# DIAGNijmegen/prostateMR_3D-CAD-csPCa

Measured on AMD Instinct MI355X. Metric: train-step volumes/sec (whole job), M1 (20,160,160,3), higher is better.
Workload: dtype bf16; 1 GPU; C3 M1 full hierarchical-probabilistic dense_skip+deep_supervision latents (3,2,1,0) (20,160,160,3); batch_per_gpu=2, global_batch=2, params=67254246, parallelism=dp1, hip_graph=True

## Files before the change

prostatemr_3d-cad-cspca_amd/csrc/conv_halo.hip:

```cpp
#include "conv_mfma.h"
#include "reduce.h"
#include <stdlib.h>
#include <stdio.h>

#define HL_MAX_XIT 10
#define HL_MAX_CH 18

struct HaloP {
    MfmaP m;
    int TW, TH, tiles_w, tiles_h, ntiles, nsplit;
    int KDs, IHt, IWt;
    int dmin, hmin, wmin;
    int sde, she, swe, pde, phe, pwe;
    int PX, spr;
    int x_slots, x_bytes;
    int nchunks, nseg, kpad;
    int b_bytes, c_bytes, stages;
    int BNh;
    int nthr;
    int tiles_per_sample;
    int spr_sh, tw_sh;
    int ncls;
    int QH, QW;
};

__device__ __forceinline__ int x_swz(int row, int sl, int spr) {
    return spr == 8 ? (sl ^ (row & 7)) : (spr == 4 ? (sl ^ ((row >> 1) & 3)) : sl);
}

__device__ __forceinline__ unsigned long long gload8_untracked(const void* p) {
    unsigned long long v;
    asm volatile("global_load_dwordx2 %0, %1, off" : "=&v"(v) : "v"(p) : "memory");
    return v;
}

template <int TN, int NTHR, int NCH, int NXIT, int B1 = 0, int B2 = 0, int B3 = 0>
__global__ void __launch_bounds__(NTHR) conv_halo_kernel(HaloP p) {
    constexpr int TM = 2, BN = TN * 16, SEG = 8, NW = NTHR / 64;
    constexpr bool RT = NCH == 0;
    constexpr bool CLS = B1 > 0;
    constexpr int NC = CLS ? 4 : 1;
    static_assert(!CLS || (NCH > 0 && B1 < B2 && B2 < B3 && B3 < NCH), "class boundaries");
#define cls_of(ch) (CLS ? ((ch) >= B1) + ((ch) >= B2) + ((ch) >= B3) : 0)
#define cls_lo(c) ((c) == 0 ? 0 : ((c) == 1 ? B1 : ((c) == 2 ? B2 : B3)))
    constexpr int CH = RT ? HL_MAX_CH : NCH, XIT = RT ? HL_MAX_XIT : NXIT;
    extern __shared__ __attribute__((aligned(16))) unsigned char smem[];
    unsigned char* const Bs = smem;
    float* const red = reinterpret_cast<float*>(smem + p.b_bytes);
    unsigned char* const Xs0 = smem + p.b_bytes + p.c_bytes;
    const MfmaP& m = p.m;
    const int tid = threadIdx.x, lane = tid & 63, wave = __builtin_amdgcn_readfirstlane(tid >> 6);
    const int oc0 = blockIdx.x * BN;
    const unsigned char* zero_pg = reinterpret_cast<const unsigned char*>(m1_zero_page);
    const int fr = lane & 15, fs = lane >> 4;
    const int spt_sh = p.spr_sh;

    {
        const bf16_t* wp = (const bf16_t*)m.wp + m.cls_woff[0];
        const int nslot = p.nchunks * BN * 4;
        for (int q0 = 0; q0 < nslot; q0 += NTHR) {
            const int q = q0 + tid;
            const int ch = q / (BN * 4), r = (q / 4) % BN, s = m1_swz64(r, q & 3);
            const unsigned char* src;
            if constexpr (CLS) {
                const int c = cls_of(ch), lo = cls_lo(c), kp = m.cls_kpad[c];
                src = (q < nslot) ? reinterpret_cast<const unsigned char*>((const bf16_t*)m.wp + m.cls_woff[c] + (long long)(oc0 + r) * kp + ((ch - lo) * 4 + s) * SEG) : zero_pg;
            } else
            src = (q < nslot) ? reinterpret_cast<const unsigned char*>(wp + (long long)(oc0 + r) * p.kpad + (ch * 4 + s) * SEG)
                                                   : zero_pg;
            if (q0 + wave * 64 < nslot) m1_glds16(src, Bs + (q0 + wave * 64) * 16);
        }
    }

    const bf16_t* x_ptr[XIT]; int x_C[XIT], x_pk[XIT];
    const int nxit = RT ? p.x_slots / NTHR : NXIT;
    const int nchunks = RT ? p.nchunks : NCH;
    const int x_rows = p.KDs * p.IHt * p.IWt;
#pragma unroll
    for (int it = 0; it < XIT; ++it) {
        const int q = it * NTHR + tid;
        const int row = q >> spt_sh, slp = q & (p.spr - 1);
        const int sl = x_swz(row, slp, p.spr);
        const int dd = row / (p.IHt * p.IWt); const int r2 = row - dd * (p.IHt * p.IWt);
        const int hh = r2 / p.IWt, ww = r2 - hh * p.IWt;
        int c = sl * SEG, s = 0;
        while (s < m.nsrc - 1 && c >= m.srcC[s]) { c -= m.srcC[s]; ++s; }
        x_C[it] = m.srcC[s];
        x_ptr[it] = (const bf16_t*)m.src[s] + (long long)((dd * m.IH + hh) * m.IW + ww) * m.srcC[s] + c;
        x_pk[it] = row < x_rows ? (dd | (hh << 8) | (ww << 16)) : -1;
    }

    int q_kt = blockIdx.y, q_tw, q_th, q_od, q_n;
    { int r = q_kt; q_tw = r % p.tiles_w; r /= p.tiles_w; q_th = r % p.tiles_h; r /= p.tiles_h; q_od = r % m.OD; q_n = r / m.OD; }
    int s_tw, s_th, s_od, s_n;
    { int r = p.nsplit; s_tw = r % p.tiles_w; r /= p.tiles_w; s_th = r % p.tiles_h; r /= p.tiles_h; s_od = r % m.OD; s_n = r / m.OD; }
    auto advance = [&](int& kt, int& tw, int& th, int& od, int& n) {
        kt += p.nsplit;
        tw += s_tw; int c = tw >= p.tiles_w; tw -= c ? p.tiles_w : 0;
        th += s_th + c; c = th >= p.tiles_h; th -= c ? p.tiles_h : 0;
        od += s_od + c; c = od >= m.OD; od -= c ? m.OD : 0;
        n += s_n + c;
    };
    auto issue = [&](int st) {
        const int live = q_kt < p.ntiles;
        const int id0 = q_od * p.sde - p.pde + p.dmin, ih0 = q_th * p.TH * p.she - p.phe + p.hmin, iw0 = q_tw * p.TW * p.swe - p.pwe + p.wmin;
        const int lin0 = ((q_n * m.ID + id0) * m.IH + ih0) * m.IW + iw0;
        unsigned char* Xs = Xs0 + st * p.x_bytes;
        const long long zp = (long long)zero_pg;
        const bool inside = live && id0 >= 0 && id0 + p.KDs <= m.ID && ih0 >= 0 && ih0 + p.IHt <= m.IH && iw0 >= 0 && iw0 + p.IWt <= m.IW;
        if (inside) {
#pragma unroll
            for (int it = 0; it < XIT; ++it) {
                if (!RT || it < nxit) {
                    const long long real = (long long)(x_ptr[it] + (long long)lin0 * x_C[it]);
                    const int ok = x_pk[it] >= 0;
                    const unsigned char* src = reinterpret_cast<const unsigned char*>(zp + ((real - zp) & -(long long)ok));
                    m1_glds16(src, Xs + (it * NTHR + wave * 64) * 16);
                }
            }
        } else {
#pragma unroll
            for (int it = 0; it < XIT; ++it) {
                if (!RT || it < nxit) {
                    const int pk = x_pk[it];
                    const int dd = pk & 0xff, hh = (pk >> 8) & 0xff, ww = (pk >> 16) & 0xff;
                    const int ok = live & (int)(pk >= 0) & (int)((unsigned)(id0 + dd) < (unsigned)m.ID) & (int)((unsigned)(ih0 + hh) < (unsigned)m.IH) &
                                   (int)((unsigned)(iw0 + ww) < (unsigned)m.IW);
                    const long long real = (long long)(x_ptr[it] + (long long)lin0 * x_C[it]);
                    const unsigned char* src = reinterpret_cast<const unsigned char*>(zp + ((real - zp) & -(long long)ok));
                    m1_glds16(src, Xs + (it * NTHR + wave * 64) * 16);
                }
            }
        }
        advance(q_kt, q_tw, q_th, q_od, q_n);
    };

    const unsigned lds0 = (unsigned)(unsigned long long)(lptr_t)smem;
    const int tw_sh = p.tw_sh;
    unsigned a_off[CH][TM];
#pragma unroll
    for (int q = 0; q < CH; ++q) {
        int kseg = q * 4 + fs, t0 = 0;
        if constexpr (CLS) {
            const int c = cls_of(q);
            kseg = (q - cls_lo(c)) * 4 + fs; t0 = m.cls_first[c];
            if (kseg >= m.cls_ntaps[c] * p.spr) kseg = 0;
        } else if (kseg >= p.nseg) kseg = 0;
        const int t = t0 + (kseg >> spt_sh), sl = kseg & (p.spr - 1);
        const int ddr = m.tdd[t] - p.dmin, dhr = m.tdh[t] - p.hmin, dwr = m.tdw[t] - p.wmin;
#pragma unroll
        for (int i = 0; i < TM; ++i) {
            const int mv = wave * 32 + i * 16 + fr;
            const int th = mv >> tw_sh, tw = mv & (p.TW - 1);
            const int row = (ddr * p.IHt + th * p.she + dhr) * p.IWt + tw * p.swe + dwr;
            a_off[q][i] = lds0 + p.b_bytes + p.c_bytes + row * p.PX + x_swz(row, sl, p.spr) * 16;
        }
    }
    unsigned b_off[TN];
#pragma unroll
    for (int j = 0; j < TN; ++j) b_off[j] = lds0 + (j * 16 + fr) * 64 + m1_swz64(fr, fs) * 16;

    int e_th[TM], e_row[TM];
#pragma unroll
    for (int i = 0; i < TM; ++i) {
        const int mv = wave * 32 + i * 16 + fr;
        e_th[i] = mv >> tw_sh; e_row[i] = CLS ? 2 * (e_th[i] * m.OW + (mv & (p.TW - 1))) : e_th[i] * m.OW + (mv & (p.TW - 1));
    }
    bf16_t* o_base[TN]; int o_C[TN], o_nv[TN], o_acc[TN], o_fast[TN]; float bias_r[TN][4];
#pragma unroll
    for (int j = 0; j < TN; ++j) {
        const int oc = oc0 + j * 16 + fs * 4;
        int nv = m.OCn - oc; nv = nv > 4 ? 4 : (nv < 0 ? 0 : nv);
        o_base[j] = nullptr; o_C[j] = 0; o_acc[j] = 0; o_fast[j] = 0;
        if (nv > 0) {
            const OutRef o = m1_out_ref(m, oc);
            if (o.base) { o_base[j] = (bf16_t*)o.base + o.col; o_C[j] = o.C; o_acc[j] = o.acc; o_fast[j] = nv == 4 && (o.C & 3) == 0 && (o.col & 3) == 0; }
            else nv = 0;
        }
        o_nv[j] = nv;
#pragma unroll
        for (int r = 0; r < 4; ++r) bias_r[j][r] = (oc + r < m.OCn) ? m1_bias_at(m, oc + r) : 0.f;
    }
#pragma unroll
    for (int j = 0; j < TN; ++j)
#pragma unroll
        for (int r = 0; r < 4; ++r) asm volatile("" : "+v"(bias_r[j][r]));
    const bool ib = !CLS && m.ib_x != nullptr;
    float* const ib_ms = red + NW * BN * 2;
    float ib_g[TN][4], ib_b[TN][4];
#pragma unroll
    for (int j = 0; j < TN; ++j)
#pragma unroll
        for (int r = 0; r < 4; ++r) {
            const int oc = oc0 + j * 16 + fs * 4 + r;
            ib_g[j][r] = (ib && oc < m.OCn) ? m.ib_gamma[oc] : 0.f; ib_b[j][r] = (ib && oc < m.OCn) ? m.ib_beta[oc] : 0.f;
        }
    if (ib) {
        for (int e = tid; e < m.N * BN; e += NTHR) {
            const int n = e / BN, c = e - n * BN, oc = oc0 + c < m.OCn ? oc0 + c : 0;
            ib_ms[e * 2] = m.ib_stats[((long long)n * m.OC + oc) * 2]; ib_ms[e * 2 + 1] = m.ib_stats[((long long)n * m.OC + oc) * 2 + 1];
        }
    }
#pragma unroll
    for (int j = 0; j < TN; ++j)
#pragma unroll
        for (int r = 0; r < 4; ++r) asm volatile("" : "+v"(ib_g[j][r]), "+v"(ib_b[j][r]));
    if (ib) { asm volatile("s_waitcnt vmcnt(0)" ::: "memory"); __syncthreads(); }
    float ssum[TN][4], ssq[TN][4];
#pragma unroll
    for (int j = 0; j < TN; ++j)
#pragma unroll
        for (int r = 0; r < 4; ++r) { ssum[j][r] = 0.f; ssq[j][r] = 0.f; }
    int cur_n = 0;
    bool any_acc = false;
#pragma unroll
    for (int j = 0; j < TN; ++j) any_acc |= o_acc[j] != 0;
    any_acc = __builtin_amdgcn_readfirstlane(__any(any_acc)) != 0;
    const bool want_stats = !CLS && m.stat_partial != nullptr;
    auto flush = [&](int n) {
#pragma unroll
        for (int j = 0; j < TN; ++j)
#pragma unroll
            for (int r = 0; r < 4; ++r) {
                float s = ssum[j][r], q = ssq[j][r];
#pragma unroll
                for (int o = 1; o < 16; o <<= 1) { s += __shfl_xor(s, o); q += __shfl_xor(q, o); }
                if (fr == 0) { red[(wave * BN + j * 16 + fs * 4 + r) * 2] = s; red[(wave * BN + j * 16 + fs * 4 + r) * 2 + 1] = q; }
                ssum[j][r] = 0.f; ssq[j][r] = 0.f;
            }
        __syncthreads();
        if (tid < BN && oc0 + tid < m.OCn) {
            float s = 0.f, q = 0.f;
            for (int w = 0; w < NW; ++w) { s += red[(w * BN + tid) * 2]; q += red[(w * BN + tid) * 2 + 1]; }
            float* dst = m.stat_partial + (((long long)n * p.nsplit + blockIdx.y) * m.OC + oc0 + tid) * 2;
            dst[0] = s; dst[1] = q;
        }
        __syncthreads();
    };

    const int S = p.stages, npiece = nxit;
    int c_kt = blockIdx.y, c_tw = q_tw, c_th = q_th, c_od = q_od, c_n = q_n;
    for (int s = 0; s < S - 1; ++s) issue(s);
    int st = 0;
    for (; c_kt < p.ntiles; advance(c_kt, c_tw, c_th, c_od, c_n)) {
        if (want_stats) { for (; cur_n < c_n; ++cur_n) flush(cur_n); }
        if constexpr (RT) m1_wait_vm<40>(npiece * (S - 2));
        else { if (S == 2) m1_wait_vm_imm<0>(); else if (S == 3) m1_wait_vm_imm<NXIT>(); else m1_wait_vm_imm<2 * NXIT>(); }
        __builtin_amdgcn_s_barrier();
        const int oh0 = c_th * p.TH;
        const int row0 = CLS ? ((c_n * m.OD + c_od) * m.OH + 2 * oh0) * m.OW + 2 * c_tw * p.TW
                             : ((c_n * m.OD + c_od) * m.OH + oh0) * m.OW + c_tw * p.TW;
        unsigned long long oldv[NC][TM][TN], xv[TM][TN];
        if (ib) {
#pragma unroll
            for (int i = 0; i < TM; ++i)
#pragma unroll
                for (int j = 0; j < TN; ++j) {
                    xv[i][j] = 0ull;
                    if (o_fast[j] && oh0 + e_th[i] < p.QH)
                        xv[i][j] = gload8_untracked((const bf16_t*)m.ib_x + (long long)(row0 + e_row[i]) * m.OC + oc0 + j * 16 + fs * 4);
                }
        }
        if (any_acc) {
#pragma unroll
            for (int c = 0; c < NC; ++c)
#pragma unroll
            for (int i = 0; i < TM; ++i)
#pragma unroll
                for (int j = 0; j < TN; ++j) {
                    oldv[c][i][j] = 0ull;
                    if (o_acc[j] && o_fast[j] && oh0 + e_th[i] < p.QH)
                        oldv[c][i][j] = gload8_untracked(o_base[j] + (long long)(row0 + e_row[i] + (c >> 1) * m.OW + (c & 1)) * o_C[j]);
                }
        }
        int stn = st + S - 1; if (stn >= S) stn -= S;
        issue(stn);
        const unsigned sb = (unsigned)(st * p.x_bytes);

        f32x4_t acc[NC][TM][TN];
#pragma unroll
        for (int c = 0; c < NC; ++c)
#pragma unroll
        for (int i = 0; i < TM; ++i)
#pragma unroll
            for (int j = 0; j < TN; ++j) acc[c][i][j] = (f32x4_t){0.f, 0.f, 0.f, 0.f};
        u32x4_t af[2][TM], bf[2][TN];
#pragma unroll
        for (int i = 0; i < TM; ++i) af[0][i] = m1_lds_read128(a_off[0][i] + sb);
#pragma unroll
        for (int j = 0; j < TN; ++j) bf[0][j] = m1_lds_read128(b_off[j]);
#pragma unroll
        for (int q = 0; q < CH; ++q) {
            if (!RT || q < nchunks) {
                const int cur = q & 1;
                m1_lds_wait(af[cur][0]);
#pragma unroll
                for (int i = 1; i < TM; ++i) m1_lds_tie(af[cur][i]);
#pragma unroll
                for (int j = 0; j < TN; ++j) m1_lds_tie(bf[cur][j]);
                if (q + 1 < CH && (!RT || q + 1 < nchunks)) {
#pragma unroll
                    for (int i = 0; i < TM; ++i) af[cur ^ 1][i] = m1_lds_read128(a_off[q + 1 < CH ? q + 1 : q][i] + sb);
#pragma unroll
                    for (int j = 0; j < TN; ++j) bf[cur ^ 1][j] = m1_lds_read128(b_off[j] + (q + 1) * BN * 64);
                }
                __builtin_amdgcn_sched_barrier(0);
#pragma unroll
                for (int i = 0; i < TM; ++i)
#pragma unroll
                    for (int j = 0; j < TN; ++j)
                        acc[cls_of(q)][i][j] = __builtin_amdgcn_mfma_f32_16x16x32_bf16(__builtin_bit_cast(bf16x8_t, bf[cur][j]),
                                                                            __builtin_bit_cast(bf16x8_t, af[cur][i]), acc[cls_of(q)][i][j], 0, 0, 0);
                __builtin_amdgcn_sched_barrier(0);
            }
        }

        if (any_acc || ib) {
            if constexpr (RT) m1_wait_vm_imm<0>(); else m1_wait_vm_imm<NXIT>();
#pragma unroll
            for (int i = 0; i < TM; ++i)
#pragma unroll
                for (int j = 0; j < TN; ++j) {
                    if (any_acc) {
#pragma unroll
                        for (int c = 0; c < NC; ++c) asm volatile("" : "+v"(oldv[c][i][j]));
// ... 62 lines not shown
    asm volatile("s_waitcnt vmcnt(0)" ::: "memory");
}
#undef cls_of
#undef cls_lo

typedef void (*halo_kern_t)(HaloP);
static halo_kern_t halo_cls_kernel(const MfmaP& mp, const HaloP& p) {
    const int nxit = p.x_slots / p.nthr;
    const int b1 = mp.cls_kpad[0] / 32, b2 = b1 + mp.cls_kpad[1] / 32, b3 = b2 + mp.cls_kpad[2] / 32;
    halo_kern_t kern = nullptr;
#define HC(NCH_, NXIT_, B1_, B2_, B3_) if (!kern && p.nchunks == NCH_ && nxit == NXIT_ && b1 == B1_ && b2 == B2_ && b3 == B3_) \
        kern = p.BNh == 32 ? conv_halo_kernel<2, 512, NCH_, NXIT_, B1_, B2_, B3_> : conv_halo_kernel<1, 512, NCH_, NXIT_, B1_, B2_, B3_>;
    HC(18, 5, 8, 12, 16) HC(18, 5, 2, 6, 10)
    HC(5, 2, 2, 3, 4) HC(5, 2, 1, 2, 3)
    HC(9, 3, 4, 6, 8) HC(9, 3, 1, 3, 5)
#undef HC
    return kern;
}
static bool halo_plan_nthr(const MfmaP& m, int OCpad, HaloP& p, int force_nthr);
static bool halo_plan(const MfmaP& m, int OCpad, HaloP& p) {
    if (halo_plan_nthr(m, OCpad, p, 0)) return true;
    return halo_plan_nthr(m, OCpad, p, 256);
}
static bool halo_plan_nthr(const MfmaP& m, int OCpad, HaloP& p, int force_nthr) {
    if (m.ksplit != 1) return false;
    const bool cls4 = m.mode == 1 && m.nclasses == 4 && m.sd == 1 && m.sh == 2 && m.sw == 2 && m.OH % 2 == 0 && m.OW % 2 == 0 &&
                      m.IH == m.OH / 2 && m.IW == m.OW / 2 && m.ID == m.OD && !m.stat_partial && !m.ib_x;
    { int hc = M1_CFG("M1_HALO_CLASSES", 1); if (cls4 && !hc) return false; }
    if (m.nclasses != 1 && !cls4) return false;
    if (!(m.mode == 0 || (m.mode == 1 && m.sd == 1 && m.sh == 1 && m.sw == 1) || cls4)) return false;
    { int hs = M1_CFG("M1_HALO_STRIDED", 1);
      if (!hs && m.mode == 0 && (m.sd > 1 || m.sh > 1 || m.sw > 1)) return false; }
    int CC = 0;
    for (int i = 0; i < m.nsrc; ++i) { if (m.srcC[i] % 8) return false; CC += m.srcC[i]; }
    if (!(CC == 8 || CC == 16 || CC == 32 || CC == 64)) return false;
    const int QH = cls4 ? m.OH / 2 : m.OH, QW = cls4 ? m.OW / 2 : m.OW;
    if (QW % 8) return false;
    if ((long long)m.N * m.ID * m.IH * m.IW >= (1ll << 31) - (1 << 20) || (long long)m.N * m.OD * m.OH * m.OW >= (1ll << 31) - (1 << 20)) return false;
    int nt = m.cls_ntaps[0];
    if (cls4) { nt = 0; for (int c = 0; c < 4; ++c) { if (m.cls_first[c] != nt) return false; nt += m.cls_ntaps[c]; } }
    if (nt < 2 || m.cls_first[0] != 0) return false;
    p = HaloP{}; p.m = m; p.ncls = cls4 ? 4 : 1; p.QH = QH; p.QW = QW;
    int dmin = 127, dmax = -127, hmin = 127, hmax = -127, wmin = 127, wmax = -127;
    for (int t = 0; t < nt; ++t) {
        dmin = m.tdd[t] < dmin ? m.tdd[t] : dmin; dmax = m.tdd[t] > dmax ? m.tdd[t] : dmax;
        hmin = m.tdh[t] < hmin ? m.tdh[t] : hmin; hmax = m.tdh[t] > hmax ? m.tdh[t] : hmax;
        wmin = m.tdw[t] < wmin ? m.tdw[t] : wmin; wmax = m.tdw[t] > wmax ? m.tdw[t] : wmax;
    }
    p.dmin = dmin; p.hmin = hmin; p.wmin = wmin;
    if (m.mode == 0) { p.sde = m.sd; p.she = m.sh; p.swe = m.sw; p.pde = m.pd; p.phe = m.ph; p.pwe = m.pw; }
    else { p.sde = p.she = p.swe = 1; p.pde = p.phe = p.pwe = 0; }
    { int nt_ = M1_CFG("M1_HALO_THREADS", 512); p.nthr = nt_ == 512 ? 512 : 256; }
    if (force_nthr) p.nthr = force_nthr;
    p.TW = QW % 32 == 0 ? 32 : (QW % 16 == 0 ? 16 : 8);
    if (p.nthr == 512) {
        const int th5 = 256 / p.TW, th2 = 128 / p.TW;
        const double e5 = (double)QH / ((QH + th5 - 1) / th5 * th5), e2 = (double)QH / ((QH + th2 - 1) / th2 * th2);
        if (e5 < 0.9 * e2) p.nthr = 256;
    }
    if (cls4 && p.nthr != 512) return false;
    const int BMh = p.nthr / 2;
    p.TH = BMh / p.TW;
    p.tiles_w = QW / p.TW; p.tiles_h = (QH + p.TH - 1) / p.TH;
    p.tiles_per_sample = m.OD * p.tiles_h * p.tiles_w;
    const long long nt_all = (long long)m.N * p.tiles_per_sample;
    if (nt_all >= (1ll << 30)) return false;
    p.ntiles = (int)nt_all;
    p.KDs = dmax - dmin + 1; p.IHt = (p.TH - 1) * p.she + (hmax - hmin + 1); p.IWt = (p.TW - 1) * p.swe + (wmax - wmin + 1);
    if (p.KDs > 255 || p.IHt > 255 || p.IWt > 255) return false;
    p.PX = CC * 2; p.spr = CC / 8;
    p.spr_sh = p.spr == 8 ? 3 : (p.spr == 4 ? 2 : (p.spr == 2 ? 1 : 0)); p.tw_sh = p.TW == 32 ? 5 : (p.TW == 16 ? 4 : 3);
    const int x_rows = p.KDs * p.IHt * p.IWt;
    p.x_slots = (x_rows * p.spr + p.nthr - 1) / p.nthr * p.nthr;
    if (p.x_slots > HL_MAX_XIT * p.nthr) return false;
    p.x_bytes = p.x_slots * 16 + 256;
    p.kpad = m.cls_kpad[0]; p.nchunks = p.kpad / 32; p.nseg = nt * p.spr;
    if (cls4) { p.kpad = 0; for (int c = 0; c < 4; ++c) p.kpad += m.cls_kpad[c]; p.nchunks = p.kpad / 32; }
    if (p.nchunks > HL_MAX_CH) return false;
    p.BNh = (m.OCn > 16 && OCpad >= 32) ? 32 : 16;
    if (OCpad % p.BNh) return false;
    p.b_bytes = p.nchunks * p.BNh * 64;
    p.c_bytes = (p.nthr / 64) * p.BNh * 2 * 4;
    if (m.ib_x) p.c_bytes += m.N * p.BNh * 2 * 4;
    const int fixed = p.b_bytes + p.c_bytes;
    int kb = M1_CFG("M1_HALO_LDS_KB", 160);
    int S = (kb * 1024 - fixed) / p.x_bytes;
    if (S > 4) S = 4;
    { int fs = M1_CFG("M1_HALO_STAGES", 0); if (fs >= 2 && fs < S) S = fs; }
    while (S > 2 && (p.x_slots / p.nthr) * (S - 2) > 40) --S;
    if (S < 2) return false;
    p.stages = S;
    if (cls4 && !halo_cls_kernel(m, p)) return false;
    return true;
}

static int halo_nsplit(const HaloP& p, int OCpad) {
    const int slices = OCpad / p.BNh;
    int nsplit = 256 / slices; if (nsplit < 1) nsplit = 1;
    { int tg = M1_CFG("M1_HALO_BLOCKS", 0); if (tg > 0) nsplit = tg / slices > 0 ? tg / slices : 1; }
    if (nsplit > p.ntiles) nsplit = p.ntiles;
    return nsplit;
}

bool m1_halo_conv_supported(const MfmaP& mp, int OCpad) { HaloP p; return halo_plan(mp, OCpad, p); }
int m1_halo_conv_stat_parts(const MfmaP& mp, int OCpad) { HaloP p; return halo_plan(mp, OCpad, p) ? halo_nsplit(p, OCpad) : 0; }

int m1_halo_conv(const MfmaP& mp, int OCpad, hipStream_t st) {
    HaloP p;
    if (!halo_plan(mp, OCpad, p)) return M1_ERR_UNSUPPORTED;
    const int slices = OCpad / p.BNh;
    const int nsplit = halo_nsplit(p, OCpad);
    p.nsplit = nsplit;
    if (mp.stat_partial && mp.stat_tiles != nsplit) return M1_ERR_BAD_ARG;
    const size_t smem = (size_t)p.b_bytes + p.c_bytes + (size_t)p.stages * p.x_bytes;
    const int nxit = p.x_slots / p.nthr;
    void (*kern)(HaloP) = nullptr;
    if (p.ncls == 4) {
        kern = halo_cls_kernel(mp, p);
        if (!kern) return M1_ERR_UNSUPPORTED;
    } else
    if (p.nthr == 512) {
#define HK(NCH_, NXIT_) if (!kern && p.nchunks == NCH_ && nxit == NXIT_) kern = p.BNh == 32 ? conv_halo_kernel<2, 512, NCH_, NXIT_> : conv_halo_kernel<1, 512, NCH_, NXIT_>;
        HK(18, 6) HK(9, 3) HK(5, 2) HK(3, 1) HK(14, 4) HK(7, 2)
#undef HK
    } else {
#define HK(NCH_, NXIT_) if (!kern && p.nchunks == NCH_ && nxit == NXIT_) kern = p.BNh == 32 ? conv_halo_kernel<2, 256, NCH_, NXIT_> : conv_halo_kernel<1, 256, NCH_, NXIT_>;
        HK(9, 9)
#undef HK
    }
    { int lg = M1_CFG("M1_HALO_LOG", 0);
      if (lg) fprintf(stderr, "halo: nthr %d BN %d nchunks %d nxit %d stages %d TW %d TH %d %s\n", p.nthr, p.BNh, p.nchunks, nxit, p.stages, p.TW, p.TH, kern ? "static" : "runtime"); }
    if (!kern) kern = p.nthr == 512 ? (p.BNh == 32 ? conv_halo_kernel<2, 512, 0, 0> : conv_halo_kernel<1, 512, 0, 0>)
                                    : (p.BNh == 32 ? conv_halo_kernel<2, 256, 0, 0> : conv_halo_kernel<1, 256, 0, 0>);
    if (m1_allow_dynamic_lds((const void*)kern, 160 * 1024) != M1_OK) return M1_ERR_LAUNCH;
    m1_note_kernel(p.ncls == 4 ? "conv_halo_cls:bn%d" : "conv_halo:bn%d", p.BNh);
    hipLaunchKernelGGL(kern, dim3(slices, nsplit), dim3(p.nthr), smem, st, p);
    return m1_check_launch();
}
```

prostatemr_3d-cad-cspca_amd/csrc/conv_mfma.h:

```cpp
#pragma once
#include "common.h"
#include "gather.h"
#include "cdna4.h"

#define MF_MAX_TAPS 27
#define MF_MAX_CLASSES 8

struct MfmaP {
    const void* src[M1_MAX_SRC];
    int srcC[M1_MAX_SRC];
    int srcSeg[M1_MAX_SRC];
    int nsrc, CC, spt;
    int ID, IH, IW;
    void* out;
    int OC, OCn;
    int nout;
    void* outs[M1_MAX_SRC]; int outC[M1_MAX_SRC]; int outOff[M1_MAX_SRC + 1]; int outAcc[M1_MAX_SRC];
    int OD, OH, OW, N;
    const void* wp;
    const float* bias;
    const float* bias2; int bias_split;
    int mode, sd, sh, sw, pd, ph, pw;
    int nclasses;
    int cls_ntaps[MF_MAX_CLASSES], cls_first[MF_MAX_CLASSES], cls_kpad[MF_MAX_CLASSES];
    long long cls_woff[MF_MAX_CLASSES];
    signed char tdd[MF_MAX_TAPS], tdh[MF_MAX_TAPS], tdw[MF_MAX_TAPS];
    int tap_pk[MF_MAX_TAPS];
    int accumulate;
    int ksplit;
    float* acc32;
    long long slab_elems;
    int aligned;
    int korder;
    const void* ib_x;
    const float* ib_stats; const float* ib_gamma; const float* ib_beta; float ib_slope;
    int tps;
    float* stat_partial;
    int stat_tiles;
};

struct OutRef { void* base; int C, col, acc; };
__device__ __forceinline__ OutRef m1_out_ref(const MfmaP& p, int oc) {
    if (p.nout == 0) return OutRef{p.out, p.OC, oc, p.accumulate};
    int m = 0;
    while (m + 1 < p.nout && oc >= p.outOff[m + 1]) ++m;
    return OutRef{p.outs[m], p.outC[m], oc - p.outOff[m], p.outAcc[m]};
}

__device__ __forceinline__ float m1_bias_at(const MfmaP& p, int oc) {
    if (p.bias_split > 0 && oc >= p.bias_split) return p.bias2 ? p.bias2[oc - p.bias_split] : 0.f;
    return p.bias ? p.bias[oc] : 0.f;
}

template <typename T> struct MT;
template <> struct MT<bf16_t> { static constexpr int SEG = 8; };
template <> struct MT<float> { static constexpr int SEG = 4; };


bool m1_halo_conv_supported(const MfmaP& mp, int OCpad);
int m1_halo_conv_stat_parts(const MfmaP& mp, int OCpad);
int m1_halo_conv(const MfmaP& mp, int OCpad, hipStream_t st);

bool m1_pw_conv_supported(const MfmaP& mp, int OCpad, int BN);
int m1_pw_conv_stat_parts(const MfmaP& mp, int OCpad, int BN);
int m1_pw_conv(const MfmaP& mp, int OCpad, int BN, hipStream_t st);
```

prostatemr_3d-cad-cspca_amd/csrc/conv_pw.hip:

```cpp
#include "conv_mfma.h"
#include "reduce.h"
#include <stdlib.h>


struct PwP {
    MfmaP m;
    int kpad, nseg;
    int nwaves;
    int V;
    long long Mtot;
};

template <int TN, int NCH>
__global__ void __launch_bounds__(256) conv_pw_kernel(PwP p) {
    constexpr int BN = TN * 16, NW = 4;
    extern __shared__ __attribute__((aligned(16))) unsigned char smem[];
    const MfmaP& m = p.m;
    const int tid = threadIdx.x, lane = tid & 63, wave = tid >> 6;
    const int fr = lane & 15, fs = lane >> 4;
    const int oc0 = blockIdx.x * BN;

    {
        const bf16_t* wp = (const bf16_t*)m.wp + m.cls_woff[0];
        for (int q = tid; q < NCH * BN * 4; q += 256) {
            const int ch = q / (BN * 4), r = (q / 4) % BN, s = q & 3;
            const uint4 v = *reinterpret_cast<const uint4*>(wp + (long long)(oc0 + r) * p.kpad + (ch * 4 + s) * 8);
            *reinterpret_cast<uint4*>(smem + ((ch * BN + r) * 4 + m1_swz64(r, s)) * 16) = v;
        }
    }
    __syncthreads();

    const bf16_t* xp[NCH]; int xC[NCH];
#pragma unroll
    for (int q = 0; q < NCH; ++q) {
        const int kseg = q * 4 + fs;
        int c = kseg * 8, s = 0;
        while (s < m.nsrc - 1 && c >= m.srcC[s]) { c -= m.srcC[s]; ++s; }
        const bool ok = kseg < p.nseg;
        xp[q] = ok ? (const bf16_t*)m.src[s] + c : nullptr; xC[q] = ok ? m.srcC[s] : 0;
    }
    bf16_t* o_base[TN]; int o_C[TN], o_nv[TN], o_acc[TN], o_fast[TN]; float bias_r[TN][4];
#pragma unroll
    for (int j = 0; j < TN; ++j) {
        const int oc = oc0 + j * 16 + fs * 4;
        int nv = m.OCn - oc; nv = nv > 4 ? 4 : (nv < 0 ? 0 : nv);
        o_base[j] = nullptr; o_C[j] = 0; o_acc[j] = 0; o_fast[j] = 0;
        if (nv > 0) {
            const OutRef o = m1_out_ref(m, oc);
            if (o.base) { o_base[j] = (bf16_t*)o.base + o.col; o_C[j] = o.C; o_acc[j] = o.acc; o_fast[j] = nv == 4 && (o.C & 3) == 0 && (o.col & 3) == 0; }
            else nv = 0;
        }
        o_nv[j] = nv;
#pragma unroll
        for (int r = 0; r < 4; ++r) bias_r[j][r] = (oc + r < m.OCn) ? m1_bias_at(m, oc + r) : 0.f;
    }
    const unsigned char* const w_rd = smem + fr * 64 + m1_swz64(fr, fs) * 16;

    const bool want_stats = m.stat_partial != nullptr;
    const bool ib = m.ib_x != nullptr;
    float ib_g[TN][4], ib_b[TN][4];
#pragma unroll
    for (int j = 0; j < TN; ++j)
#pragma unroll
        for (int r = 0; r < 4; ++r) {
            const int oc = oc0 + j * 16 + fs * 4 + r;
            ib_g[j][r] = (ib && oc < m.OCn) ? m.ib_gamma[oc] : 0.f; ib_b[j][r] = (ib && oc < m.OCn) ? m.ib_beta[oc] : 0.f;
        }
    float ssum[TN][4], ssq[TN][4];
#pragma unroll
    for (int j = 0; j < TN; ++j)
#pragma unroll
        for (int r = 0; r < 4; ++r) { ssum[j][r] = 0.f; ssq[j][r] = 0.f; }
    const int part = blockIdx.y * NW + wave;
    int cur_n = 0;
    auto flush = [&](int n) {
#pragma unroll
        for (int j = 0; j < TN; ++j)
#pragma unroll
            for (int r = 0; r < 4; ++r) {
                float s = ssum[j][r], q = ssq[j][r];
#pragma unroll
                for (int o = 1; o < 16; o <<= 1) { s += __shfl_xor(s, o); q += __shfl_xor(q, o); }
                const int oc = oc0 + j * 16 + fs * 4 + r;
                if (fr == 0 && oc < m.OCn) {
                    float* dst = m.stat_partial + (((long long)n * p.nwaves + part) * m.OC + oc) * 2;
                    dst[0] = s; dst[1] = q;
                }
                ssum[j][r] = 0.f; ssq[j][r] = 0.f;
            }
    };

    const long long step = (long long)p.nwaves * 32;
    u32x4_t xf[2][NCH], xn[2][NCH];
    auto fetch = [&](long long v0, u32x4_t (&x)[2][NCH]) {
#pragma unroll
        for (int i = 0; i < 2; ++i) {
            const long long v = v0 + i * 16 + fr;
#pragma unroll
            for (int q = 0; q < NCH; ++q) {
                x[i][q] = (u32x4_t){0u, 0u, 0u, 0u};
                if (v < p.Mtot && xp[q]) x[i][q] = *reinterpret_cast<const u32x4_t*>(xp[q] + v * xC[q]);
            }
        }
    };
    fetch((long long)part * 32, xf);
    for (long long v0 = (long long)part * 32; v0 < p.Mtot; v0 += step) {
        if (want_stats) { const int n = (int)(v0 / p.V); for (; cur_n < n; ++cur_n) flush(cur_n); }
        fetch(v0 + step, xn);
        bool vok[2];
#pragma unroll
        for (int i = 0; i < 2; ++i) vok[i] = v0 + i * 16 + fr < p.Mtot;
        f32x4_t acc[2][TN];
#pragma unroll
        for (int i = 0; i < 2; ++i)
#pragma unroll
            for (int j = 0; j < TN; ++j) acc[i][j] = (f32x4_t){0.f, 0.f, 0.f, 0.f};
#pragma unroll
        for (int q = 0; q < NCH; ++q)
#pragma unroll
            for (int j = 0; j < TN; ++j) {
                const u32x4_t wf = *reinterpret_cast<const u32x4_t*>(w_rd + (q * BN + j * 16) * 64);
#pragma unroll
                for (int i = 0; i < 2; ++i)
                    acc[i][j] = __builtin_amdgcn_mfma_f32_16x16x32_bf16(__builtin_bit_cast(bf16x8_t, wf), __builtin_bit_cast(bf16x8_t, xf[i][q]), acc[i][j], 0, 0, 0);
            }
#pragma unroll
        for (int i = 0; i < 2; ++i) {
            if (!vok[i]) continue;
            const long long orow = v0 + i * 16 + fr;
#pragma unroll
            for (int j = 0; j < TN; ++j) {
                if (o_nv[j] == 0) continue;
                bf16_t* dst = o_base[j] + orow * o_C[j];
                float v[4];
#pragma unroll
                for (int r = 0; r < 4; ++r) v[r] = acc[i][j][r] + bias_r[j][r];
                if (o_fast[j]) {
                    if (o_acc[j]) {
                        const uint2 ov = *reinterpret_cast<const uint2*>(dst);
                        const unsigned r01 = m1_cvt_pk_bf16(v[0], v[1]), r23 = m1_cvt_pk_bf16(v[2], v[3]);
                        v[0] = __uint_as_float(r01 << 16) + __uint_as_float(ov.x << 16); v[1] = __uint_as_float(r01 & 0xffff0000u) + __uint_as_float(ov.x & 0xffff0000u);
                        v[2] = __uint_as_float(r23 << 16) + __uint_as_float(ov.y << 16); v[3] = __uint_as_float(r23 & 0xffff0000u) + __uint_as_float(ov.y & 0xffff0000u);
                    }
                    uint2 o;
                    o.x = m1_cvt_pk_bf16(v[0], v[1]); o.y = m1_cvt_pk_bf16(v[2], v[3]);
                    *reinterpret_cast<uint2*>(dst) = o;
                    if (want_stats) {
                        const float r0 = __uint_as_float(o.x << 16), r1 = __uint_as_float(o.x & 0xffff0000u);
                        const float r2 = __uint_as_float(o.y << 16), r3 = __uint_as_float(o.y & 0xffff0000u);
                        if (ib) {
                            const int oc = oc0 + j * 16 + fs * 4, n = (int)(orow / p.V);
                            const float* msp = m.ib_stats + ((long long)n * m.OC + oc) * 2;
                            const float4 ms0 = *reinterpret_cast<const float4*>(msp), ms1 = *reinterpret_cast<const float4*>(msp + 4);
                            const uint2 xw = *reinterpret_cast<const uint2*>((const bf16_t*)m.ib_x + orow * m.OC + oc);
                            const float x0 = (__uint_as_float(xw.x << 16) - ms0.x) * ms0.y, x1 = (__uint_as_float(xw.x & 0xffff0000u) - ms0.z) * ms0.w;
                            const float x2 = (__uint_as_float(xw.y << 16) - ms1.x) * ms1.y, x3 = (__uint_as_float(xw.y & 0xffff0000u) - ms1.z) * ms1.w;
                            const float d0 = r0 * lrelu_g(ib_g[j][0] * x0 + ib_b[j][0], m.ib_slope), d1 = r1 * lrelu_g(ib_g[j][1] * x1 + ib_b[j][1], m.ib_slope);
                            const float d2 = r2 * lrelu_g(ib_g[j][2] * x2 + ib_b[j][2], m.ib_slope), d3 = r3 * lrelu_g(ib_g[j][3] * x3 + ib_b[j][3], m.ib_slope);
                            ssum[j][0] += d0; ssq[j][0] += d0 * x0; ssum[j][1] += d1; ssq[j][1] += d1 * x1;
                            ssum[j][2] += d2; ssq[j][2] += d2 * x2; ssum[j][3] += d3; ssq[j][3] += d3 * x3;
                        } else {
                        ssum[j][0] += r0; ssq[j][0] += r0 * r0; ssum[j][1] += r1; ssq[j][1] += r1 * r1;
                        ssum[j][2] += r2; ssq[j][2] += r2 * r2; ssum[j][3] += r3; ssq[j][3] += r3 * r3;
                        }
                    }
                } else {
#pragma unroll
                    for (int r = 0; r < 4; ++r)
                        if (r < o_nv[j]) {
                            float a = v[r];
                            if (o_acc[j]) a = bf2f(f2bf(a)) + bf2f(dst[r]);
                            const bf16_t e = f2bf(a); dst[r] = e;
                            const float vr = bf2f(e); ssum[j][r] += vr; ssq[j][r] += vr * vr;
                        }
                }
            }
        }
    #pragma unroll
        for (int i = 0; i < 2; ++i)
#pragma unroll
            for (int q = 0; q < NCH; ++q) xf[i][q] = xn[i][q];
    }
    if (want_stats) { for (; cur_n < m.N; ++cur_n) flush(cur_n); }
}

static bool pw_plan(const MfmaP& m, int OCpad, int BN, PwP& p) {
    int en = M1_CFG("M1_PW", 1);
    if (!en) return false;
    if (m.nclasses != 1 || m.ksplit != 1 || m.cls_ntaps[0] != 1) return false;
    if (m.tdd[0] != 0 || m.tdh[0] != 0 || m.tdw[0] != 0) return false;
    if (m.sd != 1 || m.sh != 1 || m.sw != 1) return false;
    if (m.ID != m.OD || m.IH != m.OH || m.IW != m.OW) return false;
    int CC = 0;
    for (int i = 0; i < m.nsrc; ++i) { if (m.srcC[i] % 8) return false; CC += m.srcC[i]; }
    const int kpad = m.cls_kpad[0];
    if (kpad % 32 || kpad / 32 > 2 || CC > kpad) return false;
    if (!(BN == 16 || BN == 32) || OCpad % BN) return false;
    p = PwP{}; p.m = m; p.kpad = kpad; p.nseg = CC / 8;
    p.V = m.OD * m.OH * m.OW; p.Mtot = (long long)m.N * p.V;
    if (p.V % 32) return false;
    return true;
}
static int pw_nwaves(const PwP& p, int OCpad, int BN) {
    const int slices = OCpad / BN;
    int tg = M1_CFG("M1_PW_BLOCKS", 2048);
    long long blocks = tg / slices; if (blocks < 1) blocks = 1;
    const long long need = (p.Mtot + 127) / 128;
    if (blocks > need) blocks = need;
    return (int)blocks * 4;
}
bool m1_pw_conv_supported(const MfmaP& mp, int OCpad, int BN) { PwP p; return pw_plan(mp, OCpad, BN, p); }
int m1_pw_conv_stat_parts(const MfmaP& mp, int OCpad, int BN) { PwP p; return pw_plan(mp, OCpad, BN, p) ? pw_nwaves(p, OCpad, BN) : 0; }

int m1_pw_conv(const MfmaP& mp, int OCpad, int BN, hipStream_t st) {
    PwP p;
    if (!pw_plan(mp, OCpad, BN, p)) return M1_ERR_UNSUPPORTED;
    p.nwaves = mp.stat_partial ? mp.stat_tiles : pw_nwaves(p, OCpad, BN);
    if (p.nwaves < 4 || p.nwaves % 4) return M1_ERR_BAD_ARG;
    const int nch = p.kpad / 32;
    const int NCH = nch <= 1 ? 1 : 2;
    if (NCH * 32 != p.kpad) {
        return M1_ERR_UNSUPPORTED;
    }
    void (*kern)(PwP) = nullptr;
#define PK(TN_, NCH_) if (BN == TN_ * 16 && NCH == NCH_) kern = conv_pw_kernel<TN_, NCH_>;
    PK(1, 1) PK(1, 2) PK(2, 1) PK(2, 2)
#undef PK
    if (!kern) return M1_ERR_UNSUPPORTED;
    const size_t smem = (size_t)NCH * BN * 64;
    if (smem > 48 * 1024 && m1_allow_dynamic_lds((const void*)kern, 64 * 1024) != M1_OK) return M1_ERR_LAUNCH;
    m1_note_kernel("conv_pw:bn%d", BN);
    hipLaunchKernelGGL(kern, dim3(OCpad / BN, p.nwaves / 4), dim3(256), smem, st, p);
    return m1_check_launch();
}
```

Baseline: 88.92 volumes/s.

## Stage kernel argument tables in LDS and issue prologue loads earlier

```diff
diff --git a/prostatemr_3d-cad-cspca_amd/csrc/conv_halo.hip b/prostatemr_3d-cad-cspca_amd/csrc/conv_halo.hip
--- a/prostatemr_3d-cad-cspca_amd/csrc/conv_halo.hip
+++ b/prostatemr_3d-cad-cspca_amd/csrc/conv_halo.hip
@@ -54,8 +54,23 @@
     const unsigned char* zero_pg = reinterpret_cast<const unsigned char*>(m1_zero_page);
     const int fr = lane & 15, fs = lane >> 4;
     const int spt_sh = p.spr_sh;
-
+    const bool ib = !CLS && m.ib_x != nullptr;
+
+    const MfmaTab* const tab = reinterpret_cast<const MfmaTab*>(smem + p.b_bytes + p.c_bytes - MF_TAB_BYTES);
+    float* const ib_ms = red + NW * BN * 2;
     {
+        const MfmaTabRow trow = m1_tab_load(m, tid, oc0, BN, ib);
+        if (ib) {
+            for (int e = tid; e < m.N * BN; e += NTHR) {
+                const int n = e / BN, c = e - n * BN, oc = oc0 + c < m.OCn ? oc0 + c : 0;
+                ib_ms[e * 2] = m.ib_stats[((long long)n * m.OC + oc) * 2]; ib_ms[e * 2 + 1] = m.ib_stats[((long long)n * m.OC + oc) * 2 + 1];
+            }
+        }
+        m1_tab_store(reinterpret_cast<MfmaTab*>(smem + p.b_bytes + p.c_bytes - MF_TAB_BYTES), trow, tid);
+    }
+    __syncthreads();
+
+    auto issue_weights = [&]() {
         const bf16_t* wp = (const bf16_t*)m.wp + m.cls_woff[0];
         const int nslot = p.nchunks * BN * 4;
         for (int q0 = 0; q0 < nslot; q0 += NTHR) {
@@ -63,14 +78,15 @@
             const int ch = q / (BN * 4), r = (q / 4) % BN, s = m1_swz64(r, q & 3);
             const unsigned char* src;
             if constexpr (CLS) {
-                const int c = cls_of(ch), lo = cls_lo(c), kp = m.cls_kpad[c];
-                src = (q < nslot) ? reinterpret_cast<const unsigned char*>((const bf16_t*)m.wp + m.cls_woff[c] + (long long)(oc0 + r) * kp + ((ch - lo) * 4 + s) * SEG) : zero_pg;
+                const int c = cls_of(ch), lo = cls_lo(c), kp = c == 0 ? m.cls_kpad[0] : (c == 1 ? m.cls_kpad[1] : (c == 2 ? m.cls_kpad[2] : m.cls_kpad[3]));
+                const long long wo = c == 0 ? m.cls_woff[0] : (c == 1 ? m.cls_woff[1] : (c == 2 ? m.cls_woff[2] : m.cls_woff[3]));
+                src = (q < nslot) ? reinterpret_cast<const unsigned char*>((const bf16_t*)m.wp + wo + (long long)(oc0 + r) * kp + ((ch - lo) * 4 + s) * SEG) : zero_pg;
             } else
             src = (q < nslot) ? reinterpret_cast<const unsigned char*>(wp + (long long)(oc0 + r) * p.kpad + (ch * 4 + s) * SEG)
                                                    : zero_pg;
             if (q0 + wave * 64 < nslot) m1_glds16(src, Bs + (q0 + wave * 64) * 16);
         }
-    }
+    };
 
     const bf16_t* x_ptr[XIT]; int x_C[XIT], x_pk[XIT];
     const int nxit = RT ? p.x_slots / NTHR : NXIT;
@@ -83,10 +99,9 @@
         const int sl = x_swz(row, slp, p.spr);
         const int dd = row / (p.IHt * p.IWt); const int r2 = row - dd * (p.IHt * p.IWt);
         const int hh = r2 / p.IWt, ww = r2 - hh * p.IWt;
-        int c = sl * SEG, s = 0;
-        while (s < m.nsrc - 1 && c >= m.srcC[s]) { c -= m.srcC[s]; ++s; }
-        x_C[it] = m.srcC[s];
-        x_ptr[it] = (const bf16_t*)m.src[s] + (long long)((dd * m.IH + hh) * m.IW + ww) * m.srcC[s] + c;
+        const int s = m1_tab_member(tab, sl * SEG), c = sl * SEG - tab->srcOff[s];
+        x_C[it] = tab->srcC[s];
+        x_ptr[it] = (const bf16_t*)m1_tab_ptr(tab->src[s]) + (long long)((dd * m.IH + hh) * m.IW + ww) * x_C[it] + c;
         x_pk[it] = row < x_rows ? (dd | (hh << 8) | (ww << 16)) : -1;
     }
 
@@ -137,17 +152,56 @@
 
     const unsigned lds0 = (unsigned)(unsigned long long)(lptr_t)smem;
     const int tw_sh = p.tw_sh;
-    unsigned a_off[CH][TM];
-#pragma unroll
-    for (int q = 0; q < CH; ++q) {
-        int kseg = q * 4 + fs, t0 = 0;
+    auto frag_kseg = [&](int q, int& t0) -> int {
+        int kseg = q * 4 + fs; t0 = 0;
         if constexpr (CLS) {
             const int c = cls_of(q);
             kseg = (q - cls_lo(c)) * 4 + fs; t0 = m.cls_first[c];
             if (kseg >= m.cls_ntaps[c] * p.spr) kseg = 0;
         } else if (kseg >= p.nseg) kseg = 0;
-        const int t = t0 + (kseg >> spt_sh), sl = kseg & (p.spr - 1);
-        const int ddr = m.tdd[t] - p.dmin, dhr = m.tdh[t] - p.hmin, dwr = m.tdw[t] - p.wmin;
+        return kseg;
+    };
+    int a_tap[CH];
+#pragma unroll
+    for (int q = 0; q < CH; ++q) { int t0; const int kseg = frag_kseg(q, t0); a_tap[q] = tab->tap[t0 + (kseg >> spt_sh)]; }
+
+    bf16_t* o_base[TN]; int o_C[TN], o_nv[TN], o_acc[TN], o_fast[TN]; float bias_r[TN][4], ib_g[TN][4], ib_b[TN][4];
+#pragma unroll
+    for (int j = 0; j < TN; ++j) {
+        const int oc = oc0 + j * 16 + fs * 4;
+        int nv = m.OCn - oc; nv = nv > 4 ? 4 : (nv < 0 ? 0 : nv);
+        o_base[j] = nullptr; o_C[j] = 0; o_acc[j] = 0; o_fast[j] = 0;
+        if (nv > 0) {
+            const OutRef o = m1_tab_out_ref(tab, oc);
+            if (o.base) { o_base[j] = (bf16_t*)o.base + o.col; o_C[j] = o.C; o_acc[j] = o.acc; o_fast[j] = nv == 4 && (o.C & 3) == 0 && (o.col & 3) == 0; }
+            else nv = 0;
+        }
+        o_nv[j] = nv;
+#pragma unroll
+        for (int r = 0; r < 4; ++r) {
+            bias_r[j][r] = tab->bias[j * 16 + fs * 4 + r]; ib_g[j][r] = tab->gamma[j * 16 + fs * 4 + r]; ib_b[j][r] = tab->beta[j * 16 + fs * 4 + r];
+        }
+    }
+#pragma unroll
+    for (int q = 0; q < CH; ++q) asm volatile("" : "+v"(a_tap[q]));
+#pragma unroll
+    for (int j = 0; j < TN; ++j) {
+        asm volatile("" : "+v"(o_C[j]), "+v"(o_acc[j]), "+v"(o_fast[j]), "+v"(o_nv[j]));
+#pragma unroll
+        for (int r = 0; r < 4; ++r) asm volatile("" : "+v"(bias_r[j][r]), "+v"(ib_g[j][r]), "+v"(ib_b[j][r]));
+    }
+
+    const int S = p.stages, npiece = nxit;
+    int c_kt = blockIdx.y, c_tw = q_tw, c_th = q_th, c_od = q_od, c_n = q_n;
+    issue_weights();
+    for (int s = 0; s < S - 1; ++s) issue(s);
+
+    unsigned a_off[CH][TM];
+#pragma unroll
+    for (int q = 0; q < CH; ++q) {
+        int t0; const int kseg = frag_kseg(q, t0);
+        const int sl = kseg & (p.spr - 1);
+        const int ddr = (int)(signed char)a_tap[q] - p.dmin, dhr = (int)(signed char)(a_tap[q] >> 8) - p.hmin, dwr = (int)(signed char)(a_tap[q] >> 16) - p.wmin;
 #pragma unroll
         for (int i = 0; i < TM; ++i) {
             const int mv = wave * 32 + i * 16 + fr;
@@ -159,53 +213,12 @@
     unsigned b_off[TN];
 #pragma unroll
     for (int j = 0; j < TN; ++j) b_off[j] = lds0 + (j * 16 + fr) * 64 + m1_swz64(fr, fs) * 16;
-
     int e_th[TM], e_row[TM];
 #pragma unroll
     for (int i = 0; i < TM; ++i) {
         const int mv = wave * 32 + i * 16 + fr;
         e_th[i] = mv >> tw_sh; e_row[i] = CLS ? 2 * (e_th[i] * m.OW + (mv & (p.TW - 1))) : e_th[i] * m.OW + (mv & (p.TW - 1));
     }
-    bf16_t* o_base[TN]; int o_C[TN], o_nv[TN], o_acc[TN], o_fast[TN]; float bias_r[TN][4];
-#pragma unroll
-    for (int j = 0; j < TN; ++j) {
-        const int oc = oc0 + j * 16 + fs * 4;
-        int nv = m.OCn - oc; nv = nv > 4 ? 4 : (nv < 0 ? 0 : nv);
-        o_base[j] = nullptr; o_C[j] = 0; o_acc[j] = 0; o_fast[j] = 0;
-        if (nv > 0) {
-            const OutRef o = m1_out_ref(m, oc);
-            if (o.base) { o_base[j] = (bf16_t*)o.base + o.col; o_C[j] = o.C; o_acc[j] = o.acc; o_fast[j] = nv == 4 && (o.C & 3) == 0 && (o.col & 3) == 0; }
-            else nv = 0;
-        }
-        o_nv[j] = nv;
-#pragma unroll
-        for (int r = 0; r < 4; ++r) bias_r[j][r] = (oc + r < m.OCn) ? m1_bias_at(m, oc + r) : 0.f;
-    }
-#pragma unroll
-    for (int j = 0; j < TN; ++j)
-#pragma unroll
-        for (int r = 0; r < 4; ++r) asm volatile("" : "+v"(bias_r[j][r]));
-    const bool ib = !CLS && m.ib_x != nullptr;
-    float* const ib_ms = red + NW * BN * 2;
-    float ib_g[TN][4], ib_b[TN][4];
-#pragma unroll
-    for (int j = 0; j < TN; ++j)
-#pragma unroll
-        for (int r = 0; r < 4; ++r) {
-            const int oc = oc0 + j * 16 + fs * 4 + r;
-            ib_g[j][r] = (ib && oc < m.OCn) ? m.ib_gamma[oc] : 0.f; ib_b[j][r] = (ib && oc < m.OCn) ? m.ib_beta[oc] : 0.f;
-        }
-    if (ib) {
-        for (int e = tid; e < m.N * BN; e += NTHR) {
-            const int n = e / BN, c = e - n * BN, oc = oc0 + c < m.OCn ? oc0 + c : 0;
-            ib_ms[e * 2] = m.ib_stats[((long long)n * m.OC + oc) * 2]; ib_ms[e * 2 + 1] = m.ib_stats[((long long)n * m.OC + oc) * 2 + 1];
-        }
-    }
-#pragma unroll
-    for (int j = 0; j < TN; ++j)
-#pragma unroll
-        for (int r = 0; r < 4; ++r) asm volatile("" : "+v"(ib_g[j][r]), "+v"(ib_b[j][r]));
-    if (ib) { asm volatile("s_waitcnt vmcnt(0)" ::: "memory"); __syncthreads(); }
     float ssum[TN][4], ssq[TN][4];
 #pragma unroll
     for (int j = 0; j < TN; ++j)
@@ -238,9 +251,6 @@
         __syncthreads();
     };
 
-    const int S = p.stages, npiece = nxit;
-    int c_kt = blockIdx.y, c_tw = q_tw, c_th = q_th, c_od = q_od, c_n = q_n;
-    for (int s = 0; s < S - 1; ++s) issue(s);
     int st = 0;
     for (; c_kt < p.ntiles; advance(c_kt, c_tw, c_th, c_od, c_n)) {
         if (want_stats) { for (; cur_n < c_n; ++cur_n) flush(cur_n); }
@@ -469,6 +479,7 @@
     p.b_bytes = p.nchunks * p.BNh * 64;
     p.c_bytes = (p.nthr / 64) * p.BNh * 2 * 4;
     if (m.ib_x) p.c_bytes += m.N * p.BNh * 2 * 4;
+    p.c_bytes += MF_TAB_BYTES;
     const int fixed = p.b_bytes + p.c_bytes;
     int kb = M1_CFG("M1_HALO_LDS_KB", 160);
     int S = (kb * 1024 - fixed) / p.x_bytes;
diff --git a/prostatemr_3d-cad-cspca_amd/csrc/conv_mfma.h b/prostatemr_3d-cad-cspca_amd/csrc/conv_mfma.h
--- a/prostatemr_3d-cad-cspca_amd/csrc/conv_mfma.h
+++ b/prostatemr_3d-cad-cspca_amd/csrc/conv_mfma.h
@@ -52,6 +52,75 @@
     return p.bias ? p.bias[oc] : 0.f;
 }
 
+#define MF_TAB_OC 32
+struct MfmaTab {
+    unsigned long long src[M1_MAX_SRC];
+    unsigned long long out[M1_MAX_SRC];
+    int srcC[M1_MAX_SRC], srcOff[M1_MAX_SRC];
+    int outC[M1_MAX_SRC], outAcc[M1_MAX_SRC];
+    int outOff[8];
+    int tap[MF_MAX_TAPS + 1];
+    int pad_[12];
+    float bias[MF_TAB_OC], gamma[MF_TAB_OC], beta[MF_TAB_OC];
+};
+#define MF_TAB_BYTES 768
+static_assert(sizeof(MfmaTab) == MF_TAB_BYTES && MF_TAB_BYTES % 128 == 0, "argument table layout");
+
+struct MfmaTabRow { unsigned long long src, out; int srcC, srcOff, outC, outAcc, outOff, tap; float bias, gamma, beta; };
+
+__device__ __forceinline__ MfmaTabRow m1_tab_load(const MfmaP& p, int tid, int oc0, int BN, bool ib) {
+    MfmaTabRow r;
+    {
+        const int l = tid & 63, i6 = l < M1_MAX_SRC ? l : M1_MAX_SRC - 1, it = l < MF_MAX_TAPS ? l : MF_MAX_TAPS - 1;
+        const bool one = p.nout == 0;
+        const unsigned long long sp = (unsigned long long)p.src[i6], op = (unsigned long long)p.outs[i6];
+        const int sC = p.srcC[i6], oC = p.outC[i6], oA = p.outAcc[i6], oO = p.outOff[i6];
+        const int td = p.tdd[it], th = p.tdh[it], tw = p.tdw[it];
+        const int oc = oc0 + l;
+        const bool live = l < BN && oc < p.OCn, second = p.bias_split > 0 && oc >= p.bias_split;
+        const float* const zp = reinterpret_cast<const float*>(m1_zero_page);
+        const float* const bsrc = second ? p.bias2 : p.bias;
+        const float* const bp = (live && bsrc) ? bsrc + (second ? oc - p.bias_split : oc) : zp;
+        const float* const gp = (live && ib) ? p.ib_gamma + oc : zp;
+        const float* const ep = (live && ib) ? p.ib_beta + oc : zp;
+        r.bias = *bp; r.gamma = *gp; r.beta = *ep;
+        int off = 0;
+#pragma unroll
+        for (int k = 0; k < M1_MAX_SRC - 1; ++k) off += k < l ? p.srcC[k] : 0;
+        r.src = sp; r.srcC = sC; r.srcOff = l < p.nsrc ? off : 0x7fffffff;
+        r.out = one ? (unsigned long long)p.out : op; r.outC = one ? p.OC : oC; r.outAcc = one ? p.accumulate : oA;
+        r.outOff = l < (one ? 1 : p.nout) ? (one ? 0 : oO) : 0x7fffffff;
+        r.tap = (td & 0xff) | ((th & 0xff) << 8) | ((tw & 0xff) << 16);
+    }
+    return r;
+}
+__device__ __forceinline__ void m1_tab_store(MfmaTab* t, MfmaTabRow r, int tid) {
+    asm volatile("" : "+v"(r.src), "+v"(r.out), "+v"(r.srcC), "+v"(r.outC), "+v"(r.outAcc), "+v"(r.outOff), "+v"(r.tap), "+v"(r.bias),
+                 "+v"(r.gamma), "+v"(r.beta));
+    if (tid < 64) {
+        const int l = tid;
+        if (l < M1_MAX_SRC) { t->src[l] = r.src; t->srcC[l] = r.srcC; t->srcOff[l] = r.srcOff; t->out[l] = r.out; t->outC[l] = r.outC; t->outAcc[l] = r.outAcc; }
+        if (l < 8) t->outOff[l] = l < M1_MAX_SRC ? r.outOff : 0x7fffffff;
+        if (l < MF_MAX_TAPS) t->tap[l] = r.tap;
+        if (l < MF_TAB_OC) { t->bias[l] = r.bias; t->gamma[l] = r.gamma; t->beta[l] = r.beta; }
+    }
+}
+__device__ __forceinline__ void* m1_tab_ptr(unsigned long long a) {
+    return (void*)reinterpret_cast<__attribute__((address_space(1))) void*>(a);
+}
+__device__ __forceinline__ int m1_tab_member(const MfmaTab* t, int c) {
+    int s = 0;
+#pragma unroll
+    for (int i = 1; i < M1_MAX_SRC; ++i) s += c >= t->srcOff[i];
+    return s;
+}
+__device__ __forceinline__ OutRef m1_tab_out_ref(const MfmaTab* t, int oc) {
+    int m = 0;
+#pragma unroll
+    for (int i = 1; i < M1_MAX_SRC; ++i) m += oc >= t->outOff[i];
+    return OutRef{m1_tab_ptr(t->out[m]), t->outC[m], oc - t->outOff[m], t->outAcc[m]};
+}
+
 template <typename T> struct MT;
 template <> struct MT<bf16_t> { static constexpr int SEG = 8; };
 template <> struct MT<float> { static constexpr int SEG = 4; };
diff --git a/prostatemr_3d-cad-cspca_amd/csrc/conv_pw.hip b/prostatemr_3d-cad-cspca_amd/csrc/conv_pw.hip
--- a/prostatemr_3d-cad-cspca_amd/csrc/conv_pw.hip
+++ b/prostatemr_3d-cad-cspca_amd/csrc/conv_pw.hip
@@ -20,6 +20,11 @@
     const int fr = lane & 15, fs = lane >> 4;
     const int oc0 = blockIdx.x * BN;
 
+    const bool want_stats = m.stat_partial != nullptr;
+    const bool ib = m.ib_x != nullptr;
+
+    const MfmaTab* const tab = reinterpret_cast<const MfmaTab*>(smem + NCH * BN * 64);
+    const MfmaTabRow trow = m1_tab_load(m, tid, oc0, BN, ib);
     {
         const bf16_t* wp = (const bf16_t*)m.wp + m.cls_woff[0];
         for (int q = tid; q < NCH * BN * 4; q += 256) {
@@ -28,17 +33,32 @@
             *reinterpret_cast<uint4*>(smem + ((ch * BN + r) * 4 + m1_swz64(r, s)) * 16) = v;
         }
     }
+    m1_tab_store(reinterpret_cast<MfmaTab*>(smem + NCH * BN * 64), trow, tid);
     __syncthreads();
 
     const bf16_t* xp[NCH]; int xC[NCH];
 #pragma unroll
     for (int q = 0; q < NCH; ++q) {
         const int kseg = q * 4 + fs;
-        int c = kseg * 8, s = 0;
-        while (s < m.nsrc - 1 && c >= m.srcC[s]) { c -= m.srcC[s]; ++s; }
+        const int s = m1_tab_member(tab, kseg * 8), c = kseg * 8 - tab->srcOff[s];
         const bool ok = kseg < p.nseg;
-        xp[q] = ok ? (const bf16_t*)m.src[s] + c : nullptr; xC[q] = ok ? m.srcC[s] : 0;
-    }
+        xp[q] = ok ? (const bf16_t*)m1_tab_ptr(tab->src[s]) + c : nullptr; xC[q] = ok ? tab->srcC[s] : 0;
+    }
+    const int part = blockIdx.y * NW + wave;
+    const long long step = (long long)p.nwaves * 32;
+    u32x4_t xf[2][NCH], xn[2][NCH];
+    auto fetch = [&](long long v0, u32x4_t (&x)[2][NCH]) {
+#pragma unroll
+        for (int i = 0; i < 2; ++i) {
+            const long long v = v0 + i * 16 + fr;
+#pragma unroll
+            for (int q = 0; q < NCH; ++q) {
+                x[i][q] = (u32x4_t){0u, 0u, 0u, 0u};
+                if (v < p.Mtot && xp[q]) x[i][q] = *reinterpret_cast<const u32x4_t*>(xp[q] + v * xC[q]);
+            }
+        }
+    };
+    fetch((long long)part * 32, xf);
     bf16_t* o_base[TN]; int o_C[TN], o_nv[TN], o_acc[TN], o_fast[TN]; float bias_r[TN][4];
 #pragma unroll
     for (int j = 0; j < TN; ++j) {
@@ -46,32 +66,26 @@
         int nv = m.OCn - oc; nv = nv > 4 ? 4 : (nv < 0 ? 0 : nv);
         o_base[j] = nullptr; o_C[j] = 0; o_acc[j] = 0; o_fast[j] = 0;
         if (nv > 0) {
-            const OutRef o = m1_out_ref(m, oc);
+            const OutRef o = m1_tab_out_ref(tab, oc);
             if (o.base) { o_base[j] = (bf16_t*)o.base + o.col; o_C[j] = o.C; o_acc[j] = o.acc; o_fast[j] = nv == 4 && (o.C & 3) == 0 && (o.col & 3) == 0; }
             else nv = 0;
         }
         o_nv[j] = nv;
 #pragma unroll
-        for (int r = 0; r < 4; ++r) bias_r[j][r] = (oc + r < m.OCn) ? m1_bias_at(m, oc + r) : 0.f;
+        for (int r = 0; r < 4; ++r) bias_r[j][r] = tab->bias[j * 16 + fs * 4 + r];
     }
     const unsigned char* const w_rd = smem + fr * 64 + m1_swz64(fr, fs) * 16;
 
-    const bool want_stats = m.stat_partial != nullptr;
-    const bool ib = m.ib_x != nullptr;
     float ib_g[TN][4], ib_b[TN][4];
 #pragma unroll
     for (int j = 0; j < TN; ++j)
 #pragma unroll
-        for (int r = 0; r < 4; ++r) {
-            const int oc = oc0 + j * 16 + fs * 4 + r;
-            ib_g[j][r] = (ib && oc < m.OCn) ? m.ib_gamma[oc] : 0.f; ib_b[j][r] = (ib && oc < m.OCn) ? m.ib_beta[oc] : 0.f;
-        }
+        for (int r = 0; r < 4; ++r) { ib_g[j][r] = tab->gamma[j * 16 + fs * 4 + r]; ib_b[j][r] = tab->beta[j * 16 + fs * 4 + r]; }
     float ssum[TN][4], ssq[TN][4];
 #pragma unroll
     for (int j = 0; j < TN; ++j)
 #pragma unroll
         for (int r = 0; r < 4; ++r) { ssum[j][r] = 0.f; ssq[j][r] = 0.f; }
-    const int part = blockIdx.y * NW + wave;
     int cur_n = 0;
     auto flush = [&](int n) {
 #pragma unroll
@@ -90,20 +104,6 @@
             }
     };
 
-    const long long step = (long long)p.nwaves * 32;
-    u32x4_t xf[2][NCH], xn[2][NCH];
-    auto fetch = [&](long long v0, u32x4_t (&x)[2][NCH]) {
-#pragma unroll
-        for (int i = 0; i < 2; ++i) {
-            const long long v = v0 + i * 16 + fr;
-#pragma unroll
-            for (int q = 0; q < NCH; ++q) {
-                x[i][q] = (u32x4_t){0u, 0u, 0u, 0u};
-                if (v < p.Mtot && xp[q]) x[i][q] = *reinterpret_cast<const u32x4_t*>(xp[q] + v * xC[q]);
-            }
-        }
-    };
-    fetch((long long)part * 32, xf);
     for (long long v0 = (long long)part * 32; v0 < p.Mtot; v0 += step) {
         if (want_stats) { const int n = (int)(v0 / p.V); for (; cur_n < n; ++cur_n) flush(cur_n); }
         fetch(v0 + step, xn);
@@ -227,7 +227,7 @@
     PK(1, 1) PK(1, 2) PK(2, 1) PK(2, 2)
 #undef PK
     if (!kern) return M1_ERR_UNSUPPORTED;
-    const size_t smem = (size_t)NCH * BN * 64;
+    const size_t smem = (size_t)NCH * BN * 64 + MF_TAB_BYTES;
     if (smem > 48 * 1024 && m1_allow_dynamic_lds((const void*)kern, 64 * 1024) != M1_OK) return M1_ERR_LAUNCH;
     m1_note_kernel("conv_pw:bn%d", BN);
     hipLaunchKernelGGL(kern, dim3(OCpad / BN, p.nwaves / 4), dim3(256), smem, st, p);
```

After: 89.61 volumes/s, median of 6. About the same (+0.8%).
